# GloireLINVANI/3D_Gaussian_Splatting_Project

Measured on AMD Instinct MI355X. Metric: Gaussians·views/sec labelled (3M G, 1080p), majority vote; first vote_view submit -> labels on the host, higher is better.
Workload: dtype f64

## Files before the change

3d_gaussian_splatting_project_amd/csrc/render.hip:

```cpp
#include <hip/hip_runtime.h>

#include <algorithm>
#include <atomic>
#include <new>
#include <thread>

#include "gsx_ctx.hpp"
#include "render_device.hpp"
#include "tile_test.hpp"

namespace gsx {

static constexpr int kScanItems = 16;
static constexpr int kScanTile = kRB * kScanItems;

__device__ __forceinline__ uint32_t block_exclusive_scan(uint32_t v, uint32_t* wsum , uint32_t& total) {
    const int lane = threadIdx.x & 63, wave = threadIdx.x >> 6;
    uint32_t inc = v;
#pragma unroll
    for (int o = 1; o < 64; o <<= 1) {
        const uint32_t up = __shfl_up(inc, o);
        if (lane >= o) inc += up;
    }
    if (lane == 63) wsum[wave] = inc;
    __syncthreads();
    uint32_t off = 0;
    for (int w = 0; w < wave; ++w) off += wsum[w];
    total = wsum[0] + wsum[1] + wsum[2] + wsum[3];
    __syncthreads();
    return off + inc - v;
}

__global__ __launch_bounds__(kRB) void scan_sums_kernel(const uint32_t* __restrict__ in, long long n,
                                                         uint32_t* __restrict__ sums) {
    __shared__ uint32_t wsum[4];
    const long long base = (long long)blockIdx.x * kScanTile + (long long)threadIdx.x * kScanItems;
    uint32_t s = 0;
#pragma unroll
    for (int k = 0; k < kScanItems; ++k)
        if (base + k < n) s += in[base + k];
    uint32_t total;
    (void)block_exclusive_scan(s, wsum, total);
    if (threadIdx.x == 0) sums[blockIdx.x] = total;
}

__global__ __launch_bounds__(kRB) void scan_down_kernel(const uint32_t* __restrict__ in, long long n,
                                                         const uint32_t* __restrict__ sums, uint32_t* __restrict__ out,
                                                         unsigned long long* __restrict__ grand) {
    __shared__ uint32_t wsum[4];
    __shared__ unsigned long long wbase[4];
    unsigned long long before = 0;
    for (int t = threadIdx.x; t < (int)blockIdx.x; t += kRB) before += sums[t];
#pragma unroll
    for (int o = 32; o > 0; o >>= 1) before += __shfl_xor(before, o);
    if ((threadIdx.x & 63) == 0) wbase[threadIdx.x >> 6] = before;
    __syncthreads();
    const unsigned long long block_base = wbase[0] + wbase[1] + wbase[2] + wbase[3];
    const long long base = (long long)blockIdx.x * kScanTile + (long long)threadIdx.x * kScanItems;
    uint32_t v[kScanItems];
    uint32_t s = 0;
#pragma unroll
    for (int k = 0; k < kScanItems; ++k) {
        v[k] = base + k < n ? in[base + k] : 0u;
        s += v[k];
    }
    uint32_t total;
    uint32_t run = (uint32_t)block_base + block_exclusive_scan(s, wsum, total);
#pragma unroll
    for (int k = 0; k < kScanItems; ++k) {
        if (base + k < n) out[base + k] = run;
        run += v[k];
    }
    if (blockIdx.x == gridDim.x - 1 && threadIdx.x == 0) *grand = block_base + total;
}

template <bool EMIT, bool BIN32>
__global__ __launch_bounds__(kRB) void bin_kernel(const unsigned long long* __restrict__ nvis_dev, long long div0, long long div1,
                                                   long long m_cap, const uint32_t* __restrict__ by_depth,
                                                   const uint32_t* __restrict__ tile_rect, const float4* __restrict__ rec,
                                                   float H, int tiles_x, int exact,
                                                   const uint8_t* __restrict__ sat, uint32_t* __restrict__ count_out,
                                                   const uint32_t* __restrict__ offset, uint32_t* __restrict__ keys,
                                                   uint32_t* __restrict__ vals, const unsigned long long* __restrict__ total_dev,
                                                   unsigned long long cap, uint32_t* __restrict__ rect_seq) {
    if (EMIT && *total_dev > cap) return;
    const long long nvis = (long long)*nvis_dev;
    const long long j0 = div0 ? nvis / div0 : 0, j1 = nvis / div1;
    const long long rel = (long long)blockIdx.x * kRB + threadIdx.x;
    const long long j = j0 + rel;
    const int lane = threadIdx.x & 63;
    const bool live = j < j1;
    const bool slot = rel < m_cap;
    const uint32_t i = live ? by_depth[j] : 0u;
    const uint32_t rect = live ? (EMIT ? rect_seq[rel] : tile_rect[i]) : kEmptyRect;
    if (!EMIT && slot) rect_seq[rel] = rect;
    const uint32_t tx0 = rect & 255u, tx1 = (rect >> 8) & 255u, ty0 = (rect >> 16) & 255u, ty1 = rect >> 24;
    constexpr uint32_t kSh = BIN32 ? 1u : 0u;
    const uint32_t w = tx1 >= tx0 ? (tx1 >> kSh) - (tx0 >> kSh) + 1u : 0u;
    const uint32_t area = w * (ty1 >= ty0 ? (ty1 >> kSh) - (ty0 >> kSh) + 1u : 0u);
    uint32_t inc = area;
#pragma unroll
    for (int o = 1; o < 64; o <<= 1) {
        const uint32_t up = __shfl_up(inc, o);
        if (lane >= o) inc += up;
    }
    const uint32_t total = __shfl(inc, 63);
    if (total == 0) {
        if (!EMIT && slot) count_out[rel] = 0u;
        return;
    }
    const uint32_t cstart = inc - area;
    if (!EMIT && !exact && !sat) {
        if (slot) count_out[rel] = area;
        return;
    }
    const bool test = exact && area > 1u;
    float4 r0 = make_float4(0.f, 0.f, 0.f, 0.f), r1 = r0;
    if (test) {
        r0 = rec[3 * (size_t)i];
        r1 = rec[3 * (size_t)i + 1];
    }
    const uint32_t my_off = EMIT && live ? offset[rel] : 0u;
    uint32_t kept_run = 0;
    for (uint32_t base = 0; base < total; base += 64u) {
        const uint32_t e = base + (uint32_t)lane;
        const bool valid = e < total;
        const uint32_t target = valid ? e : total - 1u;
        int lo = 0, hi = 63;
#pragma unroll
        for (int step = 0; step < 6; ++step) {
            const int mid = (lo + hi + 1) >> 1;
            const uint32_t om = __shfl(cstart, mid);
            if (om <= target) lo = mid;
            else hi = mid - 1;
        }
        const uint32_t s_start = __shfl(cstart, lo);
        const uint32_t s_rect = __shfl(rect, lo);
        const uint32_t s_tx0 = s_rect & 255u, s_tx1 = (s_rect >> 8) & 255u, s_ty0 = (s_rect >> 16) & 255u;
        const uint32_t s_w = (s_tx1 >> kSh) - (s_tx0 >> kSh) + 1u;
        const uint32_t local = target - s_start;
        const uint32_t ry = local / s_w, rx = local - ry * s_w;
        const uint32_t tx = (s_tx0 >> kSh) + rx, ty = (s_ty0 >> kSh) + ry;
        const uint32_t tile = ty * (uint32_t)tiles_x + tx;
        bool keep = valid;
        uint32_t tag = 0u;
        if (BIN32) {
            const uint32_t s_ty1 = s_rect >> 24;
            const uint32_t cx = 2u * tx, cy = 2u * ty;
            const uint32_t xb = (cx >= s_tx0 && cx <= s_tx1 ? 1u : 0u) | (cx + 1u >= s_tx0 && cx + 1u <= s_tx1 ? 2u : 0u);
            uint32_t m = (cy >= s_ty0 && cy <= s_ty1 ? xb : 0u) | (cy + 1u >= s_ty0 && cy + 1u <= s_ty1 ? xb << 2 : 0u);
            if (sat && keep) {
                const uint32_t sw = reinterpret_cast<const uint32_t*>(sat)[tile];
                m &= ~((sw & 0xffu ? 1u : 0u) | (sw & 0xff00u ? 2u : 0u) | (sw & 0xff0000u ? 4u : 0u) | (sw & 0xff000000u ? 8u : 0u));
            }
            keep = keep && m != 0u;
            tag = m << 28;
        }
        if (exact) {
            const int s_test = __shfl((int)test, lo);
            const float a0 = __shfl(r0.x, lo), a1 = __shfl(r0.y, lo), a2 = __shfl(r0.z, lo), a3 = __shfl(r0.w, lo);
            const float b0 = __shfl(r1.x, lo), b1 = __shfl(r1.y, lo);
            if (keep && s_test) keep = tile_touches(a0, a1, a2, a3, b0, b1, H, tx, ty);
        }
        if (!BIN32 && sat && keep) keep = sat[tile] == 0;
        if (EMIT && !exact && !sat) {
            const uint32_t pos = __shfl(my_off, lo) + local;
            const uint32_t s_i = __shfl(i, lo);
            if (keep) {
                keys[pos] = tile;
                vals[pos] = s_i | tag;
            }
            continue;
        }
        const unsigned long long verdict = __ballot(keep);
        const long long mlo = (long long)cstart - (long long)base, mhi = mlo + (long long)area;
        const int blo = (int)(mlo < 0 ? 0 : (mlo > 64 ? 64 : mlo)), bhi = (int)(mhi < 0 ? 0 : (mhi > 64 ? 64 : mhi));
        const unsigned long long below_hi = bhi >= 64 ? ~0ull : ((1ull << bhi) - 1ull);
        const unsigned long long below_lo = blo >= 64 ? ~0ull : ((1ull << blo) - 1ull);
        const uint32_t mine = (uint32_t)__popcll(verdict & below_hi & ~below_lo);
        if (EMIT) {
            const uint32_t s_prior = __shfl(kept_run, lo);
            const uint32_t s_off = __shfl(my_off, lo);
            const uint32_t s_i = __shfl(i, lo);
            const long long slo = (long long)s_start - (long long)base;
            const int sblo = (int)(slo < 0 ? 0 : slo);
            const unsigned long long upto = (1ull << lane) - 1ull;
            const unsigned long long from = sblo >= 64 ? ~0ull : ((1ull << sblo) - 1ull);
            const uint32_t rank = s_prior + (uint32_t)__popcll(verdict & upto & ~from);
            if (keep) {
                keys[s_off + rank] = tile;
                vals[s_off + rank] = s_i | tag;
            }
        }
        kept_run += mine;
    }
    if (!EMIT && slot) count_out[rel] = kept_run;
}

__global__ __launch_bounds__(kRB) void ranges_kernel(const uint32_t* __restrict__ keys, const unsigned long long* __restrict__ total,
                                                      unsigned long long cap, int ntiles, int2* __restrict__ ranges) {
    const unsigned long long tot = *total;
    const long long P = tot > cap ? 0 : (long long)tot;
    const long long p = (long long)blockIdx.x * kRB + threadIdx.x;
    if (p >= P) return;
    const uint32_t t = keys[p];
    if (t >= (uint32_t)ntiles) return;
    if (p == 0 || keys[p - 1] != t) ranges[t].x = (int)p;
    if (p == P - 1 || keys[p + 1] != t) ranges[t].y = (int)(p + 1);
}

static int exclusive_scan_u32(Ctx* c, const uint32_t* in, uint32_t* out, long long n, unsigned long long* grand_dev) {
    const int m = (int)((n + kScanTile - 1) / kScanTile);
    GSX_HIP(c, c->frame.scan.ensure(sizeof(uint32_t) * (size_t)(m + 1)));
    uint32_t* sums = c->frame.scan.as<uint32_t>();
    {
        ProfScope ps(c, "scan");
        hipLaunchKernelGGL(scan_sums_kernel, dim3(m), dim3(kRB), 0, c->stream, in, n, sums);
        hipLaunchKernelGGL(scan_down_kernel, dim3(m), dim3(kRB), 0, c->stream, in, n, sums, out, grand_dev);
    }
    GSX_HIP(c, hipGetLastError());
    return GSX_OK;
}

int debug_exclusive_scan(Ctx* c, const uint32_t* in, uint32_t* out, long long n, unsigned long long* grand_dev) {
    return exclusive_scan_u32(c, in, out, n, grand_dev);
}

int debug_ranges(Ctx* c, const uint32_t* keys, const unsigned long long* total_dev, long long cap, int nlists, int2* ranges) {
    GSX_HIP(c, hipMemsetAsync(ranges, 0, sizeof(int2) * (size_t)nlists, c->stream));
    hipLaunchKernelGGL(ranges_kernel, dim3(grid_for(cap)), dim3(kRB), 0, c->stream, keys, total_dev, (unsigned long long)cap, nlists, ranges);
    GSX_HIP(c, hipGetLastError());
    return GSX_OK;
}

static int launch_bin_phase(Ctx* c, const BinPhaseArgs& a) {
    const int lists_x = a.bin32 ? (a.tiles_x + 1) / 2 : a.tiles_x;
    const auto count_k = a.bin32 ? bin_kernel<false, true> : bin_kernel<false, false>;
    const auto emit_k = a.bin32 ? bin_kernel<true, true> : bin_kernel<true, false>;
    const long long m = a.m_cap;
    {
        ProfScope ps(c, "render_bin_count");
        hipLaunchKernelGGL(count_k, dim3(grid_for(m)), dim3(kRB), 0, c->stream,
                           a.nvis_dev, a.div0, a.div1, m, a.by_depth, a.tile_rect, a.rec, (float)a.H, lists_x,
                           a.exact, a.sat, a.count, (const uint32_t*)nullptr,
                           (uint32_t*)nullptr, (uint32_t*)nullptr, (const unsigned long long*)nullptr, 0ull, a.rect_seq);
    }
    GSX_HIP(c, hipGetLastError());
    const int rc = exclusive_scan_u32(c, a.count, a.offset, m, a.total_dev);
    if (rc) return rc;
    {
        ProfScope ps(c, "render_bin_emit");
        hipLaunchKernelGGL(emit_k, dim3(grid_for(m)), dim3(kRB), 0, c->stream,
                           a.nvis_dev, a.div0, a.div1, m, a.by_depth, a.tile_rect, a.rec, (float)a.H, lists_x,
                           a.exact, a.sat, (uint32_t*)nullptr, a.offset,
                           a.keys, a.vals, a.total_dev, a.pair_cap, a.rect_seq);
    }
    GSX_HIP(c, hipGetLastError());
    return GSX_OK;
}

int debug_bin(Ctx* c, const BinPhaseArgs& a) { return launch_bin_phase(c, a); }

int frame_plan(Ctx* c, int W, int H, bool allow_bin32, int phases, FramePlan& fp) {
    const int tiles_x = (W + 15) / 16, tiles_y = (H + 15) / 16;
    RenderFrame& f = c->frame;
    const RenderOpts& o = c->ropt;
    const int ntiles = tiles_x * tiles_y;
    const long long n = c->scene.rn;
    const bool bin32 = allow_bin32 && o.bin32 && o.blend_pk2 == 2 && !o.exact_cull && n < (1ll << 28);
    f.bin32 = bin32;
    const int bins_x = (tiles_x + 1) / 2, bins_y = (tiles_y + 1) / 2;
    const int nlists = bin32 ? bins_x * bins_y : ntiles;
    const size_t sat_bytes = bin32 ? 4 * (size_t)nlists : (size_t)ntiles;
    fp.W = W, fp.H = H, fp.tiles_x = tiles_x, fp.tiles_y = tiles_y, fp.ntiles = ntiles, fp.nlists = nlists;
    fp.bin32 = bin32, fp.sat_bytes = sat_bytes, fp.n = n;
    GSX_HIP(c, f.ranges.ensure(sizeof(int2) * (size_t)nlists));
    GSX_HIP(c, f.sat.ensure(sat_bytes));
    GSX_HIP(c, f.small.ensure(sizeof(FrameCounters)));
    f.P = 0;
    f.consumed = 0;
    if (n <= 0) return GSX_OK;
    const size_t n4 = 4 * (size_t)n;
    fp.ext_pre = f.pre_ext >= 0;
    f.cur = &f.sets[fp.ext_pre ? f.pre_ext : 0];
    int rc = ensure_pre_set(c, *f.cur, n);
    if (rc) return rc;
    GSX_HIP(c, f.bucket.ensure(n4));
    GSX_HIP(c, f.count.ensure(n4));
    GSX_HIP(c, f.offset.ensure(n4));
    GSX_HIP(c, f.d0.ensure(n4));
    GSX_HIP(c, f.d1.ensure(n4));
    GSX_HIP(c, f.d2.ensure(n4));
    GSX_HIP(c, f.d3.ensure(n4));
    GSX_HIP(c, f.rects.ensure(n4));
    const int K = std::max(1, std::min(phases, kMaxPhases));
    const long long ratio = std::max(2, std::min(o.phase_ratio, 64));
    long long* divs = fp.divs;
    divs[0] = 0;
    for (int p = 1; p <= K; ++p) {
        long long div = 1;
        for (int q = p; q < K; ++q) div = std::min<long long>(div * ratio, (long long)1 << 40);
        divs[p] = div;
    }
    int tile_bits = 1;
    while ((1 << tile_bits) < nlists) ++tile_bits;
    const bool wide = tile_bits <= 11 && (o.wide_sort == 2 || (o.wide_sort == 1 && !f.in_flight));
    if (f.pair_cap == 0) f.pair_cap = std::max<size_t>((size_t)1 << 20, 2 * (size_t)n);
    fp.K = K, fp.tile_bits = tile_bits, fp.wide = wide;
    return GSX_OK;
}

int frame_depth_order(Ctx* c, const gsx_camera* cam, FramePlan& fp) {
    RenderFrame& f = c->frame;
    const RenderOpts& o = c->ropt;
    FrameCounters* fc = f.small.as<FrameCounters>();
    const long long n = fp.n;
    int rc;
    const size_t cap = f.pair_cap;
    GSX_HIP(c, f.keys0.ensure(4 * cap));
    GSX_HIP(c, f.keys1.ensure(4 * cap));
    GSX_HIP(c, f.vals0.ensure(4 * cap));
    GSX_HIP(c, f.vals1.ensure(4 * cap));
    GSX_HIP(c, hipMemsetAsync(f.sat.p, 0, fp.sat_bytes, c->stream));
    GSX_HIP(c, hipMemsetAsync(fc, 0, sizeof(FrameCounters), c->stream));
    if (!fp.ext_pre && (rc = launch_pre(c, cam, fp.W, fp.H, *f.cur))) return rc;
    launch_bucket(c, *f.cur, f.bucket.as<uint32_t>(), f.d0.as<uint32_t>(), f.d1.as<uint32_t>(), &fc->dropped, o.compact);
    GSX_HIP(c, hipGetLastError());
    int dwhere = 0;
    rc = radix_sort_pairs_drop(c, f.d0.as<uint32_t>(), f.d1.as<uint32_t>(), f.d2.as<uint32_t>(), f.d3.as<uint32_t>(), n, nullptr, 16,
                               &dwhere, &fc->nvis);
    if (rc) return rc;
    fp.by_depth = dwhere ? f.d3.as<uint32_t>() : f.d1.as<uint32_t>();
    return GSX_OK;
}

int frame_phase_lists(Ctx* c, const FramePlan& fp, int p, int first_phase, const uint32_t** vals_sorted) {
    RenderFrame& f = c->frame;
    const RenderOpts& o = c->ropt;
    FrameCounters* fc = f.small.as<FrameCounters>();
    const size_t cap = f.pair_cap;
    const int nlists = fp.nlists;
    const bool wide = fp.wide;
    int rc;
    const long long m = fp.n / fp.divs[p + 1];
    unsigned long long* pairs_dev = &fc->pairs[p];
    int where = 0;
    if (m > 0) {
        const BinPhaseArgs bin = {&fc->nvis, fp.divs[p], fp.divs[p + 1], m, fp.by_depth, f.cur->rect.as<uint32_t>(), f.cur->rec.as<float4>(),
                                  fp.H, fp.tiles_x, fp.bin32, o.exact_cull, first_phase ? nullptr : f.sat.as<uint8_t>(),
                                  f.count.as<uint32_t>(), f.offset.as<uint32_t>(), f.rects.as<uint32_t>(), f.keys0.as<uint32_t>(),
                                  f.vals0.as<uint32_t>(), pairs_dev, (unsigned long long)cap};
        if ((rc = launch_bin_phase(c, bin))) return rc;
        if (wide) {
            rc = radix_sort_values_wide(c, f.keys0.as<uint32_t>(), f.vals0.as<uint32_t>(), f.vals1.as<uint32_t>(), (long long)cap,
                                        pairs_dev, fp.tile_bits, f.ranges.as<int2>(), nlists);
            where = 1;
        } else {
            rc = radix_sort_pairs_dev(c, f.keys0.as<uint32_t>(), f.vals0.as<uint32_t>(), f.keys1.as<uint32_t>(), f.vals1.as<uint32_t>(),
                                      (long long)cap, pairs_dev, fp.tile_bits, &where);
        }
        if (rc) return rc;
    }
    if (!(wide && m > 0)) GSX_HIP(c, hipMemsetAsync(f.ranges.p, 0, sizeof(int2) * (size_t)nlists, c->stream));
    if (m > 0 && !wide) {
        ProfScope ps(c, "render_ranges");
        hipLaunchKernelGGL(ranges_kernel, dim3(grid_for((long long)cap)), dim3(kRB), 0, c->stream,
                           where ? f.keys1.as<uint32_t>() : f.keys0.as<uint32_t>(), pairs_dev, (unsigned long long)cap, nlists,
                           f.ranges.as<int2>());
        GSX_HIP(c, hipGetLastError());
    }
    *vals_sorted = where ? f.vals1.as<uint32_t>() : f.vals0.as<uint32_t>();
    return GSX_OK;
}

int render_view(Ctx* c, const gsx_camera* cam, int W, int H, float* rgba_out) {
    GSX_HIP(c, hipSetDevice(c->device));
    if (!cam || W < 1 || H < 1) return fail(c, GSX_E_INVALID, "render_view: bad arguments");
    const int tiles_x = (W + 15) / 16, tiles_y = (H + 15) / 16;
    if (tiles_x > 256 || tiles_y > 256)
        return fail(c, GSX_E_UNSUPPORTED, "render_view: %dx%d exceeds 4096 pixels per side", W, H);
    RenderFrame& f = c->frame;
    const size_t img_bytes = sizeof(float) * 4 * (size_t)W * H;
    GSX_HIP(c, f.image.ensure(img_bytes));
    FramePlan fp;
    int rc = frame_plan(c, W, H, true, c->ropt.phases, fp);
    if (rc) return rc;
    FrameCounters* fc = f.small.as<FrameCounters>();
    const long long n = fp.n;
    if (n <= 0) {
        GSX_HIP(c, hipMemsetAsync(f.image.p, 0, img_bytes, c->stream));
        if (rgba_out) GSX_HIP(c, hipMemcpyAsync(rgba_out, f.image.p, img_bytes, hipMemcpyDeviceToHost, c->stream));
        GSX_HIP(c, hipStreamSynchronize(c->stream));
        return GSX_OK;
    }
    const int K = fp.K;

    for (int attempt = 0;; ++attempt) {
        const size_t cap = f.pair_cap;
        if ((rc = frame_depth_order(c, cam, fp))) return rc;
        int first_phase = 1;
        for (int p = 0; p < K; ++p) {
            const bool last = p == K - 1;
            if (n / fp.divs[p + 1] <= 0 && !last) continue;
            const uint32_t* vals = nullptr;
            if ((rc = frame_phase_lists(c, fp, p, first_phase, &vals))) return rc;
            rc = launch_blend(c, vals, W, H, tiles_x, tiles_y, &fc->dropped,
                              &fc->consumed[0].n, f.sat.as<uint8_t>(), first_phase, last ? 1 : 0);
            if (rc) return rc;
            first_phase = 0;
        }
        FrameCounters stats;
        GSX_HIP(c, hipMemcpyAsync(&stats, fc, sizeof stats, hipMemcpyDeviceToHost, c->stream));
        GSX_HIP(c, hipStreamSynchronize(c->stream));
        unsigned long long maxP = 0, sumP = 0;
        for (int p = 0; p < K; ++p) {
            maxP = std::max(maxP, stats.pairs[p]);
            sumP += stats.pairs[p];
        }
        if (maxP > 0x7fffffffull)
            return fail(c, GSX_E_RANGE, "render_view: %llu (tile, splat) pairs in one depth phase exceed 2^31-1 "
                                        "(a close-up of a very large scene): raise the option \"render_phases\"", maxP);
        if (maxP > cap) {
            if (attempt >= 2) return fail(c, GSX_E_STATE, "render_view: pair buffers overflowed three times in a row");
            f.pair_cap = (size_t)(maxP + maxP / 4 + 4096);
            continue;
        }
        f.P = sumP;
        f.consumed = 0;
        for (const FrameCounters::Slot& slot : stats.consumed) f.consumed += slot.n;
        break;
    }
    if (rgba_out) {
        GSX_HIP(c, hipMemcpyAsync(rgba_out, f.image.p, img_bytes, hipMemcpyDeviceToHost, c->stream));
        GSX_HIP(c, hipStreamSynchronize(c->stream));
    }
    return GSX_OK;
}

static int twin_sync_scene(Ctx* c, int k) {
    if (!c->twins[k]) {
        c->twins[k] = new (std::nothrow) Ctx();
        if (!c->twins[k]) return fail(c, GSX_E_INVALID, "render_views: out of host memory");
        c->twins[k]->device = c->device;
        hipError_t e = hipSuccess;
        if (k == 0 && c->ropt.share_stream) {
            if (second_stream(c) != GSX_OK) e = hipErrorUnknown;
            c->twins[k]->stream = c->stream2;
            c->twins[k]->stream_borrowed = true;
        } else {
            e = hipStreamCreateWithFlags(&c->twins[k]->stream, hipStreamNonBlocking);
        }
        if (e != hipSuccess) {
            c->twins[k]->stream = nullptr;
            delete c->twins[k];
            c->twins[k] = nullptr;
            return fail(c, GSX_E_HIP, "render_views: hipStreamCreate failed: %s", hipGetErrorString(e));
        }
    }
    Ctx* t = c->twins[k];
    t->scene.alias(c->scene);
    t->ropt = c->ropt;
    if (t->frame.pair_cap < c->frame.pair_cap) t->frame.pair_cap = c->frame.pair_cap;
    return GSX_OK;
}

void render_release_twin(Ctx* c) {
    for (Ctx*& t : c->twins) {
        if (!t) continue;
        (void)hipStreamSynchronize(t->stream);
        if (!t->stream_borrowed) (void)hipStreamDestroy(t->stream);
        t->stream = nullptr;
        delete t;
        t = nullptr;
    }
}

int render_views(Ctx* c, int n, const gsx_camera* cams, int W, int H, float* const* rgba_out) {
    if (n < 0 || (n > 0 && !cams)) return fail(c, GSX_E_INVALID, "render_views: bad arguments");
    if (n == 0) return GSX_OK;
    const int F = std::max(1, std::min({c->ropt.frames, kMaxFrames, n}));
    if (F == 1 || c->prof_on)
    {
        unsigned long long P = 0, used = 0;
        for (int k = 0; k < n; ++k) {
            const int rc = render_view(c, cams + k, W, H, rgba_out ? rgba_out[k] : nullptr);
            if (rc) return rc;
            P += c->frame.P;
            used += c->frame.consumed;
        }
        c->frame.P = P;
        c->frame.consumed = used;
        return GSX_OK;
    }
    int rc = GSX_OK;
    for (int f = 1; f < F; ++f)
        if ((rc = twin_sync_scene(c, f - 1))) return rc;
    int rcs[kMaxFrames] = {};
    unsigned long long P[kMaxFrames] = {}, used[kMaxFrames] = {};
    const bool multi = c->ropt.multi_pre != 0 && c->scene.rn > 0;
    const int groups = (n + F - 1) / F;
    std::atomic<int> pre_issued{0}, done[kMaxFrames];
    std::atomic<bool> failed{false};
    for (auto& d : done) d.store(0);
    Ctx* ctxs[kMaxFrames] = {c};
    for (int f = 1; f < F; ++f) ctxs[f] = c->twins[f - 1];
    if (multi) {
        for (int f = 0; f < F; ++f)
            for (PreSet& ps : ctxs[f]->frame.sets)
                if ((rc = ensure_pre_set(c, ps, c->scene.rn))) return rc;
    }
    auto issue_pre = [&](int g) -> int {
        for (int f = 0; f < F; ++f)
            while (done[f].load(std::memory_order_acquire) < std::min(g - 2, (n - 1 - f) / F + 1) && !failed.load()) std::this_thread::yield();
        if (failed.load()) return GSX_OK;
        const int set = g % kPreSets;
        const int nv = std::min(F, n - g * F);
        PreSet* sets[kMaxFrames];
        for (int v = 0; v < nv; ++v) sets[v] = &ctxs[v]->frame.sets[set];
        const int rcp = launch_pre_multi(c, nv, cams + g * F, W, H, sets, set);
        if (rcp) return rcp;
        GSX_HIP(c, c->r_pre_ev[set].record(c->stream));
        pre_issued.store(g + 1, std::memory_order_release);
        return GSX_OK;
    };
    auto frames_of = [&](Ctx* t, int f) {
        t->frame.in_flight = true;
        int g = 0;
        for (int k = f; k < n && rcs[f] == GSX_OK; k += F, ++g) {
            if (multi) {
                if (f == 0) {
                    if (g + 1 < groups && (rcs[f] = issue_pre(g + 1))) break;
                    if (failed.load()) break;
                } else {
                    while (pre_issued.load(std::memory_order_acquire) < g + 1 && !failed.load()) std::this_thread::yield();
                    if (failed.load()) break;
                    const hipError_t e = c->r_pre_ev[g % kPreSets].stream_wait(t->stream);
                    if (e != hipSuccess) {
                        rcs[f] = fail(t, GSX_E_HIP, "render_views: hipStreamWaitEvent: %s", hipGetErrorString(e));
                        break;
                    }
                }
                t->frame.pre_ext = g % kPreSets;
            }
            rcs[f] = render_view(t, cams + k, W, H, rgba_out ? rgba_out[k] : nullptr);
            t->frame.pre_ext = -1;
            P[f] += t->frame.P;
            used[f] += t->frame.consumed;
            done[f].store(g + 1, std::memory_order_release);
        }
        t->frame.pre_ext = -1;
        t->frame.in_flight = false;
        if (rcs[f] != GSX_OK) failed.store(true);
    };
    if (multi && (rc = issue_pre(0))) return rc;
    std::thread others[kMaxFrames - 1];
    int started = 0;
    try {
        for (int f = 1; f < F; ++f) {
            Ctx* t = c->twins[f - 1];
            others[f - 1] = std::thread([&, t, f] {
                try {
                    (void)hipSetDevice(t->device);
                    frames_of(t, f);
                } catch (...) {
                    rcs[f] = fail(t, GSX_E_INVALID, "render_views: a stream's host thread failed (out of host memory?)");
                    failed.store(true);
                }
            });
            ++started;
        }
        frames_of(c, 0);
    } catch (...) {
        failed.store(true);
        for (int f = 0; f < started; ++f) others[f].join();
        throw;
    }
    for (int f = 0; f < started; ++f) others[f].join();
    for (int f = 0; f < F; ++f) ctxs[f]->frame.in_flight = false;
    rc = rcs[0];
    for (int f = 1; f < F && rc == GSX_OK; ++f)
        if (rcs[f] != GSX_OK) {
            c->err = c->twins[f - 1]->err;
            rc = rcs[f];
        }
    c->frame.P = 0;
    c->frame.consumed = 0;
    for (int f = 0; f < F; ++f) {
        c->frame.P += P[f];
        c->frame.consumed += used[f];
    }
    return rc;
}

}
```

3d_gaussian_splatting_project_amd/csrc/sort.hip:

```cpp
#include <hip/hip_runtime.h>

#include <algorithm>

#include <cmath>
#include <algorithm>

#include "gsx_ctx.hpp"

namespace gsx {

static constexpr int kSortBlock = 256;
static constexpr int kSortWaves = kSortBlock / 64;
#ifndef GSX_SORT_ITEMS
#define GSX_SORT_ITEMS 16
#endif
static constexpr int kSortItems = GSX_SORT_ITEMS;
static constexpr int kSortTile = kSortBlock * kSortItems;
static constexpr int kWaveChunk = 64 * kSortItems;
static constexpr uint32_t kSortDropKey = 0xffffffffu;

__device__ __forceinline__ long long actual_count(long long n, const unsigned long long* __restrict__ n_dev) {
    if (!n_dev) return n;
    const unsigned long long v = *n_dev;
    return v > (unsigned long long)n ? 0 : (long long)v;
}

template <bool DROP>
__global__ __launch_bounds__(kSortBlock) void radix_hist_kernel(const uint32_t* __restrict__ keys, long long n,
                                                                 const unsigned long long* __restrict__ n_dev, int shift,
                                                                 uint32_t mask, uint32_t* __restrict__ hist, int ntiles) {
    __shared__ uint32_t h[256];
    n = actual_count(n, n_dev);
    if ((long long)blockIdx.x * kSortTile >= n) return;
    h[threadIdx.x] = 0;
    __syncthreads();
    const long long base = (long long)blockIdx.x * kSortTile;
#pragma unroll 4
    for (int k = 0; k < kSortItems; ++k) {
        const long long i = base + (long long)k * kSortBlock + threadIdx.x;
        if (i < n) {
            const uint32_t k = keys[i];
            if (!DROP || k != kSortDropKey) atomicAdd(&h[(k >> shift) & mask], 1u);
        }
    }
    __syncthreads();
    hist[(long long)threadIdx.x * ntiles + blockIdx.x] = h[threadIdx.x];
}

__global__ __launch_bounds__(kSortBlock) void radix_rowscan_kernel(uint32_t* __restrict__ hist, int ntiles, long long n,
                                                                    const unsigned long long* __restrict__ n_dev,
                                                                    uint32_t* __restrict__ rowsum) {
    __shared__ uint32_t wsum[kSortWaves];
    __shared__ uint32_t carry_s;
    uint32_t* row = hist + (long long)blockIdx.x * ntiles;
    ntiles = (int)((actual_count(n, n_dev) + kSortTile - 1) / kSortTile);
    const int lane = threadIdx.x & 63, wave = threadIdx.x >> 6;
    if (threadIdx.x == 0) carry_s = 0;
    __syncthreads();
    for (int t0 = 0; t0 < ntiles; t0 += kSortBlock) {
        const int t = t0 + threadIdx.x;
        const uint32_t v = t < ntiles ? row[t] : 0u;
        uint32_t inc = v;
#pragma unroll
        for (int o = 1; o < 64; o <<= 1) {
            const uint32_t up = __shfl_up(inc, o);
            if (lane >= o) inc += up;
        }
        if (lane == 63) wsum[wave] = inc;
        __syncthreads();
        uint32_t off = carry_s;
        for (int w = 0; w < wave; ++w) off += wsum[w];
        if (t < ntiles) row[t] = off + inc - v;
        __syncthreads();
        if (threadIdx.x == kSortBlock - 1) carry_s = off + inc;
        __syncthreads();
    }
    if (threadIdx.x == 0) rowsum[blockIdx.x] = carry_s;
}

template <bool DROP>
__global__ __launch_bounds__(kSortBlock) void radix_scatter_kernel(const uint32_t* __restrict__ keys_in,
                                                                    const uint32_t* __restrict__ vals_in,
                                                                    uint32_t* __restrict__ keys_out,
                                                                    uint32_t* __restrict__ vals_out, long long n,
                                                                    const unsigned long long* __restrict__ n_dev, int shift,
                                                                    uint32_t mask, const uint32_t* __restrict__ hist,
                                                                    const uint32_t* __restrict__ rowsum, int ntiles,
                                                                    unsigned long long* __restrict__ n_out) {
    __shared__ uint32_t tile_kept;
    __shared__ uint32_t gbase[256];
    __shared__ uint32_t dstart[256];
    __shared__ uint32_t wcount[kSortWaves][256];
    __shared__ uint32_t wsum[kSortWaves];
    __shared__ uint32_t sk[kSortTile];
    __shared__ uint32_t sv[kSortTile];
    const int lane = threadIdx.x & 63, wave = threadIdx.x >> 6;
    const int d = threadIdx.x;
    n = actual_count(n, n_dev);
    if ((long long)blockIdx.x * kSortTile >= n) return;

    {
        const uint32_t v = rowsum[d];
        uint32_t inc = v;
#pragma unroll
        for (int o = 1; o < 64; o <<= 1) {
            const uint32_t up = __shfl_up(inc, o);
            if (lane >= o) inc += up;
        }
        if (lane == 63) wsum[wave] = inc;
#pragma unroll
        for (int w = 0; w < kSortWaves; ++w) wcount[w][d] = 0;
        __syncthreads();
        uint32_t off = 0;
        for (int w = 0; w < wave; ++w) off += wsum[w];
        gbase[d] = off + inc - v + hist[(long long)d * ntiles + blockIdx.x];
        if (DROP && blockIdx.x == 0 && d == kSortBlock - 1) *n_out = off + inc;
    }
    __syncthreads();

    const long long tile_base = (long long)blockIdx.x * kSortTile;
    const long long wbase_idx = tile_base + (long long)wave * kWaveChunk;
    const unsigned long long lt = (1ull << lane) - 1ull;
    uint32_t key[kSortItems];
    uint32_t val[kSortItems];
    uint32_t rank[kSortItems];
#pragma unroll
    for (int r = 0; r < kSortItems; ++r) {
        const long long i = wbase_idx + r * 64 + lane;
        bool valid = i < n;
        key[r] = valid ? keys_in[i] : 0u;
        val[r] = valid ? vals_in[i] : 0u;
        if (DROP) valid = valid && key[r] != kSortDropKey;
        const uint32_t dg = (key[r] >> shift) & mask;
        unsigned long long peers = __ballot(valid);
#pragma unroll
        for (int b = 0; b < 8; ++b) {
            const unsigned long long m = __ballot((dg >> b) & 1u);
            peers &= ((dg >> b) & 1u) ? m : ~m;
        }
        const uint32_t before = wcount[wave][dg];
        rank[r] = before + (uint32_t)__popcll(peers & lt);
        if (valid && (peers & lt) == 0ull) wcount[wave][dg] = before + (uint32_t)__popcll(peers);
    }
    __syncthreads();
    {
        uint32_t tot = 0;
#pragma unroll
        for (int w = 0; w < kSortWaves; ++w) tot += wcount[w][d];
        uint32_t inc = tot;
#pragma unroll
        for (int o = 1; o < 64; o <<= 1) {
            const uint32_t up = __shfl_up(inc, o);
            if (lane >= o) inc += up;
        }
        __syncthreads();
        if (lane == 63) wsum[wave] = inc;
        __syncthreads();
        uint32_t off = 0;
        for (int w = 0; w < wave; ++w) off += wsum[w];
        uint32_t run = off + inc - tot;
        dstart[d] = run;
        if (d == kSortBlock - 1) tile_kept = off + inc;
#pragma unroll
        for (int w = 0; w < kSortWaves; ++w) {
            const uint32_t c = wcount[w][d];
            wcount[w][d] = run;
            run += c;
        }
    }
    __syncthreads();
#pragma unroll
    for (int r = 0; r < kSortItems; ++r) {
        const long long i = wbase_idx + r * 64 + lane;
        if (i < n && (!DROP || key[r] != kSortDropKey)) {
            const uint32_t dg = (key[r] >> shift) & mask;
            const uint32_t lpos = wcount[wave][dg] + rank[r];
            sk[lpos] = key[r];
            sv[lpos] = val[r];
        }
    }
    __syncthreads();
    const int count = (int)tile_kept;
    for (int j = threadIdx.x; j < count; j += kSortBlock) {
        const uint32_t k = sk[j];
        const uint32_t dg = (k >> shift) & mask;
        const uint32_t pos = gbase[dg] + ((uint32_t)j - dstart[dg]);
        keys_out[pos] = k;
        vals_out[pos] = sv[j];
    }
}

int radix_sort_pairs(Ctx* c, uint32_t* k0, uint32_t* v0, uint32_t* k1, uint32_t* v1, long long n, int bits,
                     int* result_in) {
    return radix_sort_pairs_dev(c, k0, v0, k1, v1, n, nullptr, bits, result_in);
}

int radix_sort_pairs_dev(Ctx* c, uint32_t* k0, uint32_t* v0, uint32_t* k1, uint32_t* v1, long long n,
                         const unsigned long long* n_dev, int bits, int* result_in) {
    return radix_sort_pairs_drop(c, k0, v0, k1, v1, n, n_dev, bits, result_in, nullptr);
}

int radix_sort_pairs_drop(Ctx* c, uint32_t* k0, uint32_t* v0, uint32_t* k1, uint32_t* v1, long long n,
                          const unsigned long long* n_dev, int bits, int* result_in, unsigned long long* n_kept) {
    *result_in = 0;
    if (n_kept && (n_dev || n <= 0 || bits <= 0)) return fail(c, GSX_E_INVALID, "radix_sort_pairs_drop: needs a host count and at least one pass");
    if ((n <= 1 && !n_dev && !n_kept) || n <= 0 || bits <= 0) return GSX_OK;
    const int ntiles = (int)((n + kSortTile - 1) / kSortTile);
    GSX_HIP(c, c->sort_hist.ensure(sizeof(uint32_t) * ((size_t)256 * ntiles + 256)));
    uint32_t* hist = c->sort_hist.as<uint32_t>();
    uint32_t* rowsum = hist + (size_t)256 * ntiles;
    uint32_t *ki = k0, *vi = v0, *ko = k1, *vo = v1;
    int where = 0;
    const int passes = (bits + 7) / 8;
    int shift = 0;
    for (int pass = 0; pass < passes; ++pass) {
        const int width = (bits - shift + (passes - pass) - 1) / (passes - pass);
        const uint32_t mask = (1u << width) - 1u;
        {
            ProfScope ps(c, "radix_hist");
            if (n_kept && pass == 0)
                hipLaunchKernelGGL(radix_hist_kernel<true>, dim3(ntiles), dim3(kSortBlock), 0, c->stream, ki, n, n_dev, shift, mask, hist, ntiles);
            else
                hipLaunchKernelGGL(radix_hist_kernel<false>, dim3(ntiles), dim3(kSortBlock), 0, c->stream, ki, n, n_dev, shift, mask, hist, ntiles);
        }
        {
            ProfScope ps(c, "radix_rowscan");
            hipLaunchKernelGGL(radix_rowscan_kernel, dim3(256), dim3(kSortBlock), 0, c->stream, hist, ntiles, n, n_dev, rowsum);
        }
        {
            ProfScope ps(c, "radix_scatter");
            if (n_kept && pass == 0)
                hipLaunchKernelGGL(radix_scatter_kernel<true>, dim3(ntiles), dim3(kSortBlock), 0, c->stream, ki, vi, ko, vo, n, n_dev,
                                   shift, mask, hist, rowsum, ntiles, n_kept);
            else
                hipLaunchKernelGGL(radix_scatter_kernel<false>, dim3(ntiles), dim3(kSortBlock), 0, c->stream, ki, vi, ko, vo, n, n_dev,
                                   shift, mask, hist, rowsum, ntiles, (unsigned long long*)nullptr);
        }
        if (n_kept && pass == 0) n_dev = n_kept;
        GSX_HIP(c, hipGetLastError());
        std::swap(ki, ko);
        std::swap(vi, vo);
        where ^= 1;
        shift += width;
    }
    *result_in = where;
    return GSX_OK;
}

static constexpr int kWideLog = 11;
static constexpr int kWideDigits = 1 << kWideLog;
static constexpr int kWidePer = kWideDigits / kSortBlock;

__global__ __launch_bounds__(kSortBlock) void wide_hist_kernel(const uint32_t* __restrict__ keys, long long n,
                                                                const unsigned long long* __restrict__ n_dev, uint32_t mask,
                                                                uint32_t* __restrict__ hist, int ntiles) {
    __shared__ uint32_t h[kWideDigits];
    n = actual_count(n, n_dev);
    if ((long long)blockIdx.x * kSortTile >= n) return;
#pragma unroll
    for (int k = 0; k < kWidePer; ++k) h[threadIdx.x + k * kSortBlock] = 0;
    __syncthreads();
    const long long base = (long long)blockIdx.x * kSortTile;
#pragma unroll 4
    for (int k = 0; k < kSortItems; ++k) {
        const long long i = base + (long long)k * kSortBlock + threadIdx.x;
        if (i < n) atomicAdd(&h[keys[i] & mask], 1u);
    }
    __syncthreads();
#pragma unroll
    for (int k = 0; k < kWidePer; ++k) {
        const int d = threadIdx.x + k * kSortBlock;
        hist[(long long)d * ntiles + blockIdx.x] = h[d];
    }
}

__global__ __launch_bounds__(kSortBlock) void wide_scatter_kernel(const uint32_t* __restrict__ keys_in,
                                                                   const uint32_t* __restrict__ vals_in,
                                                                   uint32_t* __restrict__ vals_out, long long n,
                                                                   const unsigned long long* __restrict__ n_dev, uint32_t mask,
                                                                   const uint32_t* __restrict__ hist,
                                                                   const uint32_t* __restrict__ rowsum, int ntiles,
                                                                   int2* __restrict__ ranges, int nranges) {
    __shared__ uint32_t gbase[kWideDigits];
    __shared__ uint32_t wcount[kSortWaves][kWideDigits];
    __shared__ uint32_t wsum[kSortWaves];
    const int lane = threadIdx.x & 63, wave = threadIdx.x >> 6;
    n = actual_count(n, n_dev);
    const bool active = (long long)blockIdx.x * kSortTile < n;
    if (!active && blockIdx.x != 0) return;
    {
        uint32_t rs[kWidePer];
        uint32_t sum = 0;
#pragma unroll
        for (int k = 0; k < kWidePer; ++k) {
            rs[k] = rowsum[threadIdx.x * kWidePer + k];
            sum += rs[k];
        }
        uint32_t inc = sum;
#pragma unroll
        for (int o = 1; o < 64; o <<= 1) {
            const uint32_t up = __shfl_up(inc, o);
            if (lane >= o) inc += up;
        }
        if (lane == 63) wsum[wave] = inc;
        __syncthreads();
        uint32_t run = inc - sum;
        for (int w = 0; w < wave; ++w) run += wsum[w];
#pragma unroll
        for (int k = 0; k < kWidePer; ++k) {
            const int d = threadIdx.x * kWidePer + k;
            if (blockIdx.x == 0 && d < nranges) ranges[d] = make_int2((int)run, (int)(run + rs[k]));
            gbase[d] = run + (active ? hist[(long long)d * ntiles + blockIdx.x] : 0u);
            run += rs[k];
#pragma unroll
            for (int w = 0; w < kSortWaves; ++w) wcount[w][d] = 0;
        }
    }
    if (!active) return;
    __syncthreads();
    const long long wbase_idx = (long long)blockIdx.x * kSortTile + (long long)wave * kWaveChunk;
    const unsigned long long lt = (1ull << lane) - 1ull;
    uint32_t dig[kSortItems];
    uint32_t val[kSortItems];
    uint32_t rank[kSortItems];
#pragma unroll
    for (int r = 0; r < kSortItems; ++r) {
        const long long i = wbase_idx + r * 64 + lane;
        const bool valid = i < n;
        const uint32_t dg = valid ? keys_in[i] & mask : 0u;
        val[r] = valid ? vals_in[i] : 0u;
        dig[r] = dg;
        unsigned long long peers = __ballot(valid);
#pragma unroll
        for (int b = 0; b < kWideLog; ++b) {
            const unsigned long long m = __ballot((dg >> b) & 1u);
            peers &= ((dg >> b) & 1u) ? m : ~m;
        }
        const uint32_t before = wcount[wave][dg];
        rank[r] = before + (uint32_t)__popcll(peers & lt);
        if (valid && (peers & lt) == 0ull) wcount[wave][dg] = before + (uint32_t)__popcll(peers);
    }
    __syncthreads();
#pragma unroll
    for (int k = 0; k < kWidePer; ++k) {
        const int d = threadIdx.x + k * kSortBlock;
        uint32_t run = 0;
#pragma unroll
        for (int w = 0; w < kSortWaves; ++w) {
            const uint32_t c = wcount[w][d];
            wcount[w][d] = run;
            run += c;
        }
    }
    __syncthreads();
#pragma unroll
    for (int r = 0; r < kSortItems; ++r) {
        const long long i = wbase_idx + r * 64 + lane;
        if (i < n) vals_out[gbase[dig[r]] + wcount[wave][dig[r]] + rank[r]] = val[r];
    }
}

int radix_sort_values_wide(Ctx* c, const uint32_t* k0, const uint32_t* v0, uint32_t* v1, long long n, const unsigned long long* n_dev,
                           int bits, int2* ranges, int nranges) {
    if (n <= 0 || bits < 1 || bits > kWideLog || nranges > kWideDigits || !ranges)
        return fail(c, GSX_E_INVALID, "radix_sort_values_wide: bad arguments");
    const int ntiles = (int)((n + kSortTile - 1) / kSortTile);
    GSX_HIP(c, c->sort_hist.ensure(sizeof(uint32_t) * ((size_t)kWideDigits * ntiles + kWideDigits)));
    uint32_t* hist = c->sort_hist.as<uint32_t>();
    uint32_t* rowsum = hist + (size_t)kWideDigits * ntiles;
    const uint32_t mask = (1u << bits) - 1u;
    {
        ProfScope ps(c, "radix_hist");
        hipLaunchKernelGGL(wide_hist_kernel, dim3(ntiles), dim3(kSortBlock), 0, c->stream, k0, n, n_dev, mask, hist, ntiles);
    }
    {
        ProfScope ps(c, "radix_rowscan");
        hipLaunchKernelGGL(radix_rowscan_kernel, dim3(kWideDigits), dim3(kSortBlock), 0, c->stream, hist, ntiles, n, n_dev, rowsum);
    }
    {
        ProfScope ps(c, "radix_scatter");
        hipLaunchKernelGGL(wide_scatter_kernel, dim3(ntiles), dim3(kSortBlock), 0, c->stream, k0, v0, v1, n, n_dev, mask, hist, rowsum,
                           ntiles, ranges, nranges);
    }
    GSX_HIP(c, hipGetLastError());
    return GSX_OK;
}

__device__ __forceinline__ float finite_or(float v, float alt) { return (v - v == 0.0f) ? v : alt; }

__global__ __launch_bounds__(kSortBlock) void bbox_partial_kernel(const float* __restrict__ x,
                                                                   const float* __restrict__ y,
                                                                   const float* __restrict__ z, long long n,
                                                                   float* __restrict__ partial ) {
    float lo[3] = {3.0e38f, 3.0e38f, 3.0e38f}, hi[3] = {-3.0e38f, -3.0e38f, -3.0e38f};
    for (long long i = (long long)blockIdx.x * kSortBlock + threadIdx.x; i < n; i += (long long)gridDim.x * kSortBlock) {
        const float v[3] = {x[i], y[i], z[i]};
#pragma unroll
        for (int a = 0; a < 3; ++a) {
            lo[a] = fminf(lo[a], finite_or(v[a], 3.0e38f));
            hi[a] = fmaxf(hi[a], finite_or(v[a], -3.0e38f));
        }
    }
    __shared__ float s[kSortWaves][6];
    const int lane = threadIdx.x & 63, wave = threadIdx.x >> 6;
#pragma unroll
    for (int a = 0; a < 3; ++a) {
#pragma unroll
        for (int o = 32; o > 0; o >>= 1) {
            lo[a] = fminf(lo[a], __shfl_xor(lo[a], o));
            hi[a] = fmaxf(hi[a], __shfl_xor(hi[a], o));
        }
        if (lane == 0) {
            s[wave][a] = lo[a];
            s[wave][3 + a] = hi[a];
        }
    }
    __syncthreads();
    if (threadIdx.x < 6) {
        float r = s[0][threadIdx.x];
        for (int w = 1; w < kSortWaves; ++w) r = threadIdx.x < 3 ? fminf(r, s[w][threadIdx.x]) : fmaxf(r, s[w][threadIdx.x]);
        partial[blockIdx.x * 6 + threadIdx.x] = r;
    }
}

__global__ void bbox_final_kernel(const float* __restrict__ partial, int nparts, float* __restrict__ box) {
    if (threadIdx.x < 6) {
        float r = partial[threadIdx.x];
        for (int p = 1; p < nparts; ++p) {
            const float v = partial[p * 6 + threadIdx.x];
            r = threadIdx.x < 3 ? fminf(r, v) : fmaxf(r, v);
        }
        box[threadIdx.x] = r;
    }
}

__device__ __forceinline__ unsigned long long spread21(unsigned long long v) {
    v &= 0x1fffffull;
    v = (v | (v << 32)) & 0x1f00000000ffffull;
    v = (v | (v << 16)) & 0x1f0000ff0000ffull;
    v = (v | (v << 8)) & 0x100f00f00f00f00full;
    v = (v | (v << 4)) & 0x10c30c30c30c30c3ull;
    return (v | (v << 2)) & 0x1249249249249249ull;
}

__global__ __launch_bounds__(kSortBlock) void morton_kernel(const float* __restrict__ x, const float* __restrict__ y,
                                                             const float* __restrict__ z, long long n,
                                                             const float* __restrict__ box,
                                                             uint32_t* __restrict__ code_lo, uint32_t* __restrict__ code_hi,
                                                             uint32_t* __restrict__ idx) {
    const long long i = (long long)blockIdx.x * kSortBlock + threadIdx.x;
    if (i >= n) return;
    const float v[3] = {x[i], y[i], z[i]};
    unsigned long long q[3];
#pragma unroll
    for (int a = 0; a < 3; ++a) {
        const double ext = (double)box[3 + a] - (double)box[a];
        double t = ext > 0.0 ? ((double)v[a] - (double)box[a]) / ext * 2097151.0 : 0.0;
        t = (t - t == 0.0) ? fmin(fmax(t, 0.0), 2097151.0) : 0.0;
        q[a] = (unsigned long long)t;
    }
    const unsigned long long code = spread21(q[0]) | (spread21(q[1]) << 1) | (spread21(q[2]) << 2);
    code_lo[i] = (uint32_t)code;
    code_hi[i] = (uint32_t)(code >> 32);
    idx[i] = (uint32_t)i;
}

__global__ __launch_bounds__(kSortBlock) void gather1_kernel(const uint32_t* __restrict__ in, const uint32_t* __restrict__ perm,
                                                              long long n, uint32_t* __restrict__ out) {
    const long long i = (long long)blockIdx.x * kSortBlock + threadIdx.x;
    if (i < n) out[i] = in[perm[i]];
}

__global__ __launch_bounds__(kSortBlock) void gather3_kernel(const float* __restrict__ x, const float* __restrict__ y,
                                                              const float* __restrict__ z,
                                                              const uint32_t* __restrict__ perm, long long n,
                                                              float* __restrict__ ox, float* __restrict__ oy,
                                                              float* __restrict__ oz) {
    const long long i = (long long)blockIdx.x * kSortBlock + threadIdx.x;
    if (i >= n) return;
    const uint32_t s = perm[i];
    ox[i] = x[s];
    oy[i] = y[s];
    oz[i] = z[s];
}

int spatial_sort_positions(Ctx* c) {
    const long long n = c->n;
    c->sorted = false;
    if (n < 2) return GSX_OK;
    const size_t nb = sizeof(uint32_t) * (size_t)n;
    DevBuf code0, code1, codeh, idx1, box, tx, ty, tz;
    GSX_HIP(c, code0.ensure(nb));
    GSX_HIP(c, code1.ensure(nb));
    GSX_HIP(c, codeh.ensure(nb));
    GSX_HIP(c, idx1.ensure(nb));
    GSX_HIP(c, c->perm.ensure(nb));
    const int parts = 512;
    GSX_HIP(c, box.ensure(sizeof(float) * (6 * parts + 6)));
    float* partial = box.as<float>();
    float* bb = partial + 6 * parts;
    const unsigned grid = (unsigned)((n + kSortBlock - 1) / kSortBlock);
    hipLaunchKernelGGL(bbox_partial_kernel, dim3(parts), dim3(kSortBlock), 0, c->stream, c->x.as<float>(), c->y.as<float>(),
                       c->z.as<float>(), n, partial);
    hipLaunchKernelGGL(bbox_final_kernel, dim3(1), dim3(64), 0, c->stream, partial, parts, bb);
    hipLaunchKernelGGL(morton_kernel, dim3(grid), dim3(kSortBlock), 0, c->stream, c->x.as<float>(), c->y.as<float>(),
                       c->z.as<float>(), n, bb, code0.as<uint32_t>(), codeh.as<uint32_t>(), c->perm.as<uint32_t>());
    GSX_HIP(c, hipGetLastError());
    uint32_t* idx[2] = {c->perm.as<uint32_t>(), idx1.as<uint32_t>()};
    int where = 0;
    int rc = radix_sort_pairs(c, code0.as<uint32_t>(), idx[0], code1.as<uint32_t>(), idx[1], n, 32, &where);
    if (!rc) {
        uint32_t* sorted_idx = idx[where];
        uint32_t* other_idx = idx[where ^ 1];
        hipLaunchKernelGGL(gather1_kernel, dim3(grid), dim3(kSortBlock), 0, c->stream, codeh.as<uint32_t>(), sorted_idx, n,
                           code0.as<uint32_t>());
        GSX_HIP(c, hipGetLastError());
        int where2 = 0;
        rc = radix_sort_pairs(c, code0.as<uint32_t>(), sorted_idx, code1.as<uint32_t>(), other_idx, n, 31, &where2);
        if (!rc) {
            uint32_t* final_idx = where2 ? other_idx : sorted_idx;
            if (final_idx != c->perm.as<uint32_t>()) {
                hipError_t e = hipMemcpyAsync(c->perm.p, final_idx, nb, hipMemcpyDeviceToDevice, c->stream);
                if (e != hipSuccess) rc = fail(c, GSX_E_HIP, "spatial sort: %s", hipGetErrorString(e));
            }
        }
    }
    if (!rc) {
        hipError_t e = tx.ensure(sizeof(float) * n);
        if (e == hipSuccess) e = ty.ensure(sizeof(float) * n);
        if (e == hipSuccess) e = tz.ensure(sizeof(float) * n);
        if (e == hipSuccess) {
            hipLaunchKernelGGL(gather3_kernel, dim3(grid), dim3(kSortBlock), 0, c->stream, c->x.as<float>(), c->y.as<float>(),
                               c->z.as<float>(), c->perm.as<uint32_t>(), n, tx.as<float>(), ty.as<float>(), tz.as<float>());
            e = hipGetLastError();
        }
        if (e == hipSuccess) e = hipStreamSynchronize(c->stream);
        if (e != hipSuccess) rc = fail(c, GSX_E_HIP, "spatial sort: %s", hipGetErrorString(e));
        else {
            std::swap(c->x, tx);
            std::swap(c->y, ty);
            std::swap(c->z, tz);
            c->sorted = true;
        }
    }
    (void)hipStreamSynchronize(c->stream);
    for (DevBuf* b : {&code0, &code1, &codeh, &idx1, &box, &tx, &ty, &tz}) b->release();
    return rc;
}

}
```

Before: 88.01 billion.

## Vectorize scan loads/stores and aggregate radix histogram atomics per wave

The two-pass scan kernels now load and store four-element vectors in a wave-striped layout, so accesses coalesce instead of each thread walking 16 contiguous elements. The down-sweep does a per-row wave scan with running carries, which removes the block-wide scan with two barriers. The radix and wide histogram kernels preload keys into registers and use a ballot so the wave's leading digit is counted with a single shared atomic, with the remaining lanes adding individually. This targets shared-atomic contention on skewed digit distributions, at the cost of extra ballot and readlane work when digits are spread out.

```diff
diff --git a/3d_gaussian_splatting_project_amd/csrc/render.hip b/3d_gaussian_splatting_project_amd/csrc/render.hip
--- a/3d_gaussian_splatting_project_amd/csrc/render.hip
+++ b/3d_gaussian_splatting_project_amd/csrc/render.hip
@@ -13,35 +13,38 @@
 
 static constexpr int kScanItems = 16;
 static constexpr int kScanTile = kRB * kScanItems;
-
-__device__ __forceinline__ uint32_t block_exclusive_scan(uint32_t v, uint32_t* wsum , uint32_t& total) {
-    const int lane = threadIdx.x & 63, wave = threadIdx.x >> 6;
-    uint32_t inc = v;
-#pragma unroll
-    for (int o = 1; o < 64; o <<= 1) {
-        const uint32_t up = __shfl_up(inc, o);
-        if (lane >= o) inc += up;
-    }
-    if (lane == 63) wsum[wave] = inc;
-    __syncthreads();
-    uint32_t off = 0;
-    for (int w = 0; w < wave; ++w) off += wsum[w];
-    total = wsum[0] + wsum[1] + wsum[2] + wsum[3];
-    __syncthreads();
-    return off + inc - v;
-}
+static constexpr int kScanRows = kScanItems / 4;
+static constexpr int kScanWave = 64 * kScanItems;
+
+__device__ __forceinline__ uint4 scan_load4(const uint32_t* __restrict__ in, long long i, long long n, bool vec) {
+    if (vec && i + 4 <= n) return *reinterpret_cast<const uint4*>(in + i);
+    uint4 v = make_uint4(0u, 0u, 0u, 0u);
+    if (i < n) v.x = in[i];
+    if (i + 1 < n) v.y = in[i + 1];
+    if (i + 2 < n) v.z = in[i + 2];
+    if (i + 3 < n) v.w = in[i + 3];
+    return v;
+}
+
+__device__ __forceinline__ bool scan_aligned(const void* p) { return (reinterpret_cast<uintptr_t>(p) & 15u) == 0; }
 
 __global__ __launch_bounds__(kRB) void scan_sums_kernel(const uint32_t* __restrict__ in, long long n,
                                                          uint32_t* __restrict__ sums) {
     __shared__ uint32_t wsum[4];
-    const long long base = (long long)blockIdx.x * kScanTile + (long long)threadIdx.x * kScanItems;
+    const int lane = threadIdx.x & 63, wave = threadIdx.x >> 6;
+    const long long wbase = (long long)blockIdx.x * kScanTile + (long long)wave * kScanWave + 4 * lane;
+    const bool vec = scan_aligned(in);
     uint32_t s = 0;
 #pragma unroll
-    for (int k = 0; k < kScanItems; ++k)
-        if (base + k < n) s += in[base + k];
-    uint32_t total;
-    (void)block_exclusive_scan(s, wsum, total);
-    if (threadIdx.x == 0) sums[blockIdx.x] = total;
+    for (int j = 0; j < kScanRows; ++j) {
+        const uint4 v = scan_load4(in, wbase + j * 256, n, vec);
+        s += v.x + v.y + v.z + v.w;
+    }
+#pragma unroll
+    for (int o = 32; o > 0; o >>= 1) s += __shfl_xor(s, o);
+    if (lane == 0) wsum[wave] = s;
+    __syncthreads();
+    if (threadIdx.x == 0) sums[blockIdx.x] = wsum[0] + wsum[1] + wsum[2] + wsum[3];
 }
 
 __global__ __launch_bounds__(kRB) void scan_down_kernel(const uint32_t* __restrict__ in, long long n,
@@ -49,29 +52,54 @@
                                                          unsigned long long* __restrict__ grand) {
     __shared__ uint32_t wsum[4];
     __shared__ unsigned long long wbase[4];
+    const int lane = threadIdx.x & 63, wave = threadIdx.x >> 6;
+    const long long base = (long long)blockIdx.x * kScanTile + (long long)wave * kScanWave + 4 * lane;
+    const bool vec_in = scan_aligned(in), vec_out = scan_aligned(out);
+    uint4 v[kScanRows];
+#pragma unroll
+    for (int j = 0; j < kScanRows; ++j) v[j] = scan_load4(in, base + j * 256, n, vec_in);
     unsigned long long before = 0;
     for (int t = threadIdx.x; t < (int)blockIdx.x; t += kRB) before += sums[t];
 #pragma unroll
     for (int o = 32; o > 0; o >>= 1) before += __shfl_xor(before, o);
-    if ((threadIdx.x & 63) == 0) wbase[threadIdx.x >> 6] = before;
+    if (lane == 0) wbase[wave] = before;
+    uint32_t excl[kScanRows];
+    uint32_t wave_run = 0;
+#pragma unroll
+    for (int j = 0; j < kScanRows; ++j) {
+        const uint32_t s = v[j].x + v[j].y + v[j].z + v[j].w;
+        uint32_t inc = s;
+#pragma unroll
+        for (int o = 1; o < 64; o <<= 1) {
+            const uint32_t up = __shfl_up(inc, o);
+            if (lane >= o) inc += up;
+        }
+        excl[j] = wave_run + inc - s;
+        wave_run += __shfl(inc, 63);
+    }
+    if (lane == 0) wsum[wave] = wave_run;
     __syncthreads();
     const unsigned long long block_base = wbase[0] + wbase[1] + wbase[2] + wbase[3];
-    const long long base = (long long)blockIdx.x * kScanTile + (long long)threadIdx.x * kScanItems;
-    uint32_t v[kScanItems];
-    uint32_t s = 0;
-#pragma unroll
-    for (int k = 0; k < kScanItems; ++k) {
-        v[k] = base + k < n ? in[base + k] : 0u;
-        s += v[k];
-    }
-    uint32_t total;
-    uint32_t run = (uint32_t)block_base + block_exclusive_scan(s, wsum, total);
-#pragma unroll
-    for (int k = 0; k < kScanItems; ++k) {
-        if (base + k < n) out[base + k] = run;
-        run += v[k];
-    }
-    if (blockIdx.x == gridDim.x - 1 && threadIdx.x == 0) *grand = block_base + total;
+    uint32_t off = (uint32_t)block_base;
+    for (int w = 0; w < wave; ++w) off += wsum[w];
+#pragma unroll
+    for (int j = 0; j < kScanRows; ++j) {
+        const long long i = base + j * 256;
+        uint4 o;
+        o.x = off + excl[j];
+        o.y = o.x + v[j].x;
+        o.z = o.y + v[j].y;
+        o.w = o.z + v[j].z;
+        if (vec_out && i + 4 <= n) {
+            *reinterpret_cast<uint4*>(out + i) = o;
+        } else {
+            if (i < n) out[i] = o.x;
+            if (i + 1 < n) out[i + 1] = o.y;
+            if (i + 2 < n) out[i + 2] = o.z;
+            if (i + 3 < n) out[i + 3] = o.w;
+        }
+    }
+    if (blockIdx.x == gridDim.x - 1 && threadIdx.x == 0) *grand = block_base + (wsum[0] + wsum[1] + wsum[2] + wsum[3]);
 }
 
 template <bool EMIT, bool BIN32>
diff --git a/3d_gaussian_splatting_project_amd/csrc/sort.hip b/3d_gaussian_splatting_project_amd/csrc/sort.hip
--- a/3d_gaussian_splatting_project_amd/csrc/sort.hip
+++ b/3d_gaussian_splatting_project_amd/csrc/sort.hip
@@ -25,6 +25,16 @@
     return v > (unsigned long long)n ? 0 : (long long)v;
 }
 
+__device__ __forceinline__ void wave_count_digit(uint32_t* __restrict__ h, uint32_t dg, bool valid, int lane) {
+    const unsigned long long live = __ballot(valid);
+    if (live == 0ull) return;
+    const int first = __ffsll((long long)live) - 1;
+    const uint32_t d0 = (uint32_t)__builtin_amdgcn_readlane((int)dg, first);
+    const unsigned long long same = __ballot(dg == d0) & live;
+    if (lane == first) atomicAdd(&h[d0], (uint32_t)__popcll(same));
+    if (((live & ~same) >> lane) & 1ull) atomicAdd(&h[dg], 1u);
+}
+
 template <bool DROP>
 __global__ __launch_bounds__(kSortBlock) void radix_hist_kernel(const uint32_t* __restrict__ keys, long long n,
                                                                  const unsigned long long* __restrict__ n_dev, int shift,
@@ -34,14 +44,19 @@
     if ((long long)blockIdx.x * kSortTile >= n) return;
     h[threadIdx.x] = 0;
     __syncthreads();
-    const long long base = (long long)blockIdx.x * kSortTile;
-#pragma unroll 4
-    for (int k = 0; k < kSortItems; ++k) {
-        const long long i = base + (long long)k * kSortBlock + threadIdx.x;
-        if (i < n) {
-            const uint32_t k = keys[i];
-            if (!DROP || k != kSortDropKey) atomicAdd(&h[(k >> shift) & mask], 1u);
-        }
+    const int lane = threadIdx.x & 63, wave = threadIdx.x >> 6;
+    const long long wbase_idx = (long long)blockIdx.x * kSortTile + (long long)wave * kWaveChunk;
+    uint32_t key[kSortItems];
+#pragma unroll
+    for (int r = 0; r < kSortItems; ++r) {
+        const long long i = wbase_idx + r * 64 + lane;
+        key[r] = i < n ? keys[i] : 0u;
+    }
+#pragma unroll
+    for (int r = 0; r < kSortItems; ++r) {
+        const long long i = wbase_idx + r * 64 + lane;
+        const bool valid = i < n && (!DROP || key[r] != kSortDropKey);
+        wave_count_digit(h, (key[r] >> shift) & mask, valid, lane);
     }
     __syncthreads();
     hist[(long long)threadIdx.x * ntiles + blockIdx.x] = h[threadIdx.x];
@@ -260,12 +275,16 @@
 #pragma unroll
     for (int k = 0; k < kWidePer; ++k) h[threadIdx.x + k * kSortBlock] = 0;
     __syncthreads();
-    const long long base = (long long)blockIdx.x * kSortTile;
-#pragma unroll 4
-    for (int k = 0; k < kSortItems; ++k) {
-        const long long i = base + (long long)k * kSortBlock + threadIdx.x;
-        if (i < n) atomicAdd(&h[keys[i] & mask], 1u);
-    }
+    const int lane = threadIdx.x & 63, wave = threadIdx.x >> 6;
+    const long long wbase_idx = (long long)blockIdx.x * kSortTile + (long long)wave * kWaveChunk;
+    uint32_t key[kSortItems];
+#pragma unroll
+    for (int r = 0; r < kSortItems; ++r) {
+        const long long i = wbase_idx + r * 64 + lane;
+        key[r] = i < n ? keys[i] : 0u;
+    }
+#pragma unroll
+    for (int r = 0; r < kSortItems; ++r) wave_count_digit(h, key[r] & mask, wbase_idx + r * 64 + lane < n, lane);
     __syncthreads();
 #pragma unroll
     for (int k = 0; k < kWidePer; ++k) {
```

Measured after the change: 87.34 billion. No clear change (-0.8%).
